# VideoVerses/VideoTuna-dev

Hardware: AMD Instinct MI355X
Metric: finetune samples/sec, CogVideoX-2B T2V LoRA 49x480x720 bf16 (higher is better)
Workload: dtype bf16; 1 GPU; CogVideoX-2B T2V LoRA finetune 49x480x720 (configs[1]): latents [4,13,16,60,90], text [4,226,4096], r=4 LoRA on to_q/k/v/out, 4 samples per optimizer step as in the YAML (batch_size 2 x accumulate_grad_batches 2), run as 1 micro-batch(es) of 4; mode=lora, model=CogVideoX-2B, micro_batch=4, accumulate_grad_batches=1, global_batch=4, seq_len=17776, layers=30, parallelism=dp1, recompute=none (107 GB of block activations kept in HBM), weights=seeded random init (no checkpoints offline), text=pre-encoded prompt embeddings (synthetic), latents=pre-encoded latents (synthetic)

## Files before the change

videotuna-dev_amd/csrc/gemm_bf16.hip:

```cpp
#include "gemm_epilogue.h"

#ifndef VT_SUFFIX
#define VT_SUFFIX
#endif
#ifndef VT_GEMM_DMA
#define VT_GEMM_DMA 1
#endif
#define VT_CAT_(a, b) a##b
#define VT_CAT(a, b) VT_CAT_(a, b)
#define GEMM_KERNEL VT_CAT(gemm_tn_kernel, VT_SUFFIX)
#define GEMM_ENTRY VT_CAT(vt_gemm_bf16, VT_SUFFIX)

#define BM 128
#define BN 128
#define BK 64
#define CS_LD 132

template <int EPI, bool OUT_F32>
__global__ __launch_bounds__(256, 2) void GEMM_KERNEL(GemmParams p) {
    __shared__ __attribute__((aligned(16))) char smem[65536];
    const int tid = threadIdx.x, lane = tid & 63, wave = tid >> 6;
    const int wm = wave & 1, wn = wave >> 1;
    const int nbm = (p.M + BM - 1) / BM, nbn = (p.N + BN - 1) / BN;
    const int id = xcd_remap(blockIdx.x, nbm * nbn);
    const int GM = 8;
    const int in_group = GM * nbn;
    const int group = id / in_group;
    const int first_m = group * GM;
    const int gsz = min(nbm - first_m, GM);
    const int tile_m = first_m + (id % in_group) % gsz;
    const int tile_n = (id % in_group) / gsz;
    const int row0 = tile_m * BM, col0 = tile_n * BN;

    const long long a_rem = (long long)(p.M - row0) * p.lda * 2;
    const long long w_rem = (long long)(p.N - col0) * p.ldw * 2;
    __amdgpu_buffer_rsrc_t ra = make_rsrc(p.A + (size_t)row0 * p.lda, (unsigned)(a_rem > 0x7fffffffLL ? 0x7fffffffLL : a_rem));
    __amdgpu_buffer_rsrc_t rw = make_rsrc(p.W + (size_t)col0 * p.ldw, (unsigned)(w_rem > 0x7fffffffLL ? 0x7fffffffLL : w_rem));

#if VT_GEMM_DMA
    const int wv = __builtin_amdgcn_readfirstlane(wave);
    const int drl = lane >> 3, dcp = lane & 7;
    int a_voff[4], w_voff[4];
#pragma unroll
    for (int j = 0; j < 4; ++j) {
        const int row = 8 * (wv + 4 * j) + drl;
        a_voff[j] = row * p.lda * 2 + ((dcp ^ drl) << 4);
        w_voff[j] = row * p.ldw * 2 + ((dcp ^ drl) << 4);
    }
    auto dma = [&](int kt, int buf) {
        const int soff = kt * BK * 2;
#pragma unroll
        for (int j = 0; j < 4; ++j) {
            char* dst = smem + buf * 32768 + (wv + 4 * j) * 1024;
            __builtin_amdgcn_raw_ptr_buffer_load_lds(ra, (__attribute__((address_space(3))) void*)dst, 16, a_voff[j], soff, 0, 0);
            __builtin_amdgcn_raw_ptr_buffer_load_lds(rw, (__attribute__((address_space(3))) void*)(dst + 16384), 16, w_voff[j], soff, 0, 0);
        }
    };
#else
    int a_voff[4], w_voff[4], lds_off[4];
#pragma unroll
    for (int j = 0; j < 4; ++j) {
        int i = tid + 256 * j;
        int r = i >> 3, c = i & 7;
        a_voff[j] = r * p.lda * 2 + c * 16;
        w_voff[j] = r * p.ldw * 2 + c * 16;
        lds_off[j] = r * 128 + ((c ^ (r & 7)) << 4);
    }
    u32x4 ga[4], gw[4];
    auto gload = [&](int kt) {
        const int soff = kt * BK * 2;
#pragma unroll
        for (int j = 0; j < 4; ++j) {
            ga[j] = __builtin_bit_cast(u32x4, __builtin_amdgcn_raw_buffer_load_b128(ra, a_voff[j], soff, 0));
            gw[j] = __builtin_bit_cast(u32x4, __builtin_amdgcn_raw_buffer_load_b128(rw, w_voff[j], soff, 0));
        }
    };
    auto lstore = [&](int buf) {
        char* base = smem + buf * 32768;
#pragma unroll
        for (int j = 0; j < 4; ++j) {
            *(u32x4*)(base + lds_off[j]) = ga[j];
            *(u32x4*)(base + 16384 + lds_off[j]) = gw[j];
        }
    };
#endif

    f32x4 acc[4][4];
#pragma unroll
    for (int i = 0; i < 4; ++i)
#pragma unroll
        for (int j = 0; j < 4; ++j) acc[i][j] = (f32x4){0.f, 0.f, 0.f, 0.f};

    const int nk = p.K / BK;
#if VT_GEMM_DMA
    dma(0, 0);
#else
    gload(0);
    lstore(0);
#endif
    __syncthreads();
    const int frow = lane & 15;
    const int fq = lane >> 4;
    const int fx = lane & 7;
    for (int kt = 0; kt < nk; ++kt) {
        const int buf = kt & 1;
#if VT_GEMM_DMA
        if (kt + 1 < nk) dma(kt + 1, buf ^ 1);
#else
        if (kt + 1 < nk) gload(kt + 1);
#endif
        const char* As = smem + buf * 32768;
        const char* Ws = As + 16384;
#pragma unroll
        for (int ks = 0; ks < 2; ++ks) {
            const int coff = (((ks * 4 + fq) ^ fx) << 4);
            bf16x8 af[4], wf[4];
#pragma unroll
            for (int t = 0; t < 4; ++t) {
                af[t] = *(const bf16x8*)(As + (wm * 64 + t * 16 + frow) * 128 + coff);
                wf[t] = *(const bf16x8*)(Ws + (wn * 64 + t * 16 + frow) * 128 + coff);
            }
#pragma unroll
            for (int tn = 0; tn < 4; ++tn)
#pragma unroll
                for (int tm = 0; tm < 4; ++tm)
                    acc[tn][tm] = __builtin_amdgcn_mfma_f32_16x16x32_bf16(wf[tn], af[tm], acc[tn][tm], 0, 0, 0);
        }
#if !VT_GEMM_DMA
        if (kt + 1 < nk) lstore(buf ^ 1);
#endif
        __syncthreads();
    }

    float* Cs = (float*)smem;
    const int er = tid >> 5;
    const int ec = (tid & 31) * 4;
    const int n = col0 + ec;
    float bias4[4] = {0.f, 0.f, 0.f, 0.f};
    if (p.bias != nullptr && n < p.N) {
#pragma unroll
        for (int j = 0; j < 4; ++j) bias4[j] = bf2f(p.bias[n + j]);
    }
#pragma unroll
    for (int half = 0; half < 2; ++half) {
        if (wm == half) {
#pragma unroll
            for (int tn = 0; tn < 4; ++tn)
#pragma unroll
                for (int tm = 0; tm < 4; ++tm) {
                    int ml = tm * 16 + frow;
                    int nl = wn * 64 + tn * 16 + fq * 4;
                    *(f32x4*)(Cs + ml * CS_LD + nl) = acc[tn][tm];
                }
        }
        __syncthreads();
#pragma unroll
        for (int pass = 0; pass < 8; ++pass) {
            const int ml = pass * 8 + er;
            const int m = row0 + half * 64 + ml;
            if (m < p.M && n < p.N) {
                f32x4 v = *(const f32x4*)(Cs + ml * CS_LD + ec);
                gemm_epilogue_store<EPI, OUT_F32>(p, m, n, v, bias4);
            }
        }
        __syncthreads();
    }
}

template <int EPI, bool F32>
static int VT_CAT(launch, VT_SUFFIX)(const GemmParams& p, hipStream_t st) {
    const int nbm = (p.M + BM - 1) / BM, nbn = (p.N + BN - 1) / BN;
    hipLaunchKernelGGL((GEMM_KERNEL<EPI, F32>), dim3(nbm * nbn), dim3(256), 0, st, p);
    return hipGetLastError() == hipSuccess ? VT_OK : VT_ERR_LAUNCH;
}

static bool VT_CAT(al16, VT_SUFFIX)(const void* p) { return (((uintptr_t)p) & 15) == 0; }

int VT_CAT(vt_gemm_big_dispatch, VT_SUFFIX)(const GemmParams& p, int epilogue, int out_fp32, hipStream_t st);
int VT_CAT(vt_gemm_pc_dispatch, VT_SUFFIX)(const GemmParams& p, int epilogue, int out_fp32, hipStream_t st);
static int VT_CAT(g_gemm_tile, VT_SUFFIX) = 0;
extern "C" int VT_CAT(vt_gemm_set_tile, VT_SUFFIX)(int mode) {
    if (mode < 0 || mode > 3) return VT_ERR_BAD_SHAPE;
    VT_CAT(g_gemm_tile, VT_SUFFIX) = mode;
    return VT_OK;
}
static int VT_CAT(pick_tile, VT_SUFFIX)(int M, int N, int K) {
    const int mode = VT_CAT(g_gemm_tile, VT_SUFFIX);
    if (mode) return mode;
    const long long t256 = (long long)((M + 255) / 256) * ((N + 255) / 256);
    const long long tpc = (long long)((M + 255) / 256) * ((N + 127) / 128);
    if (N >= 6144 && t256 >= 512) return 2;
    if (K >= 512 && M >= 1024) {
        const long long passes = (t256 + 255) / 256;
        const bool full = t256 <= 256 ? t256 >= 160 : 10 * t256 >= 9 * passes * 256;
        if (full && (N >= 2560 || ((N % 640) == 0 && N <= 1280) || ((N % 256) >= 192 && K >= 4096))) return 2;
    }
    if (tpc >= 512 && K >= 512) return 3;
    if (M > 64 && M <= 1024 && (long long)N * K >= (1LL << 24)) return 3;
    return 1;
}

int VT_CAT(vt_gemm_pc_bm, VT_SUFFIX)(int M);
extern "C" int VT_CAT(vt_gemm_bf16_kernel, VT_SUFFIX)(int M, int N, int K) {
    if (M <= 0 || N <= 0 || K <= 0) return VT_ERR_BAD_SHAPE;
    const int tile = VT_CAT(pick_tile, VT_SUFFIX)(M, N, K);
    return tile == 3 && VT_CAT(vt_gemm_pc_bm, VT_SUFFIX)(M) == 128 ? 4 : tile;
}

extern "C" int GEMM_ENTRY(const void* A, int lda, const void* W, int ldw, void* C, int ldc,
                            int M, int N, int K, const void* bias, int epilogue, int out_fp32,
                            const void* R, int ldr, int r_mod,
                            const float* gate_txt, const float* gate_vid, int gate_bstride, int S, int St,
                            void* C2, int ldc2, const void* U, int ldu, void* stream) {
    if (M <= 0 || N <= 0 || K <= 0 || (K % BK) != 0 || (N % 4) != 0) return VT_ERR_BAD_SHAPE;
    if ((lda % 8) || (ldw % 8) || (ldc % 4) || lda < K || ldw < K || ldc < N) return VT_ERR_BAD_SHAPE;
    if (!VT_CAT(al16, VT_SUFFIX)(A) || !VT_CAT(al16, VT_SUFFIX)(W) || !VT_CAT(al16, VT_SUFFIX)(C)) return VT_ERR_BAD_ALIGN;
    GemmParams p;
    p.A = (const bf16_t*)A; p.W = (const bf16_t*)W; p.C = C; p.bias = (const bf16_t*)bias;
    p.R = (const bf16_t*)R; p.gate_txt = gate_txt; p.gate_vid = gate_vid;
    p.C2 = (bf16_t*)C2; p.U = (const bf16_t*)U;
    p.M = M; p.N = N; p.K = K; p.lda = lda; p.ldw = ldw; p.ldc = ldc; p.ldr = ldr; p.ldc2 = ldc2; p.ldu = ldu;
    p.S = S > 0 ? S : 1; p.St = St; p.gate_bstride = gate_bstride; p.r_mod = r_mod; p.splits = 1;
    hipStream_t st = (hipStream_t)stream;
    const int tile = VT_CAT(pick_tile, VT_SUFFIX)(M, N, K);
    const bool big = tile == 2;
    if (tile == 3) {
        if (epilogue == EPI_BIAS_GELU && (out_fp32 || C2 == nullptr || (ldc2 % 4) || !VT_CAT(al16, VT_SUFFIX)(C2))) return VT_ERR_BAD_SHAPE;
        if (epilogue == EPI_GATED_RES && (out_fp32 || R == nullptr || (ldr % 4) || !VT_CAT(al16, VT_SUFFIX)(R))) return VT_ERR_BAD_SHAPE;
        if (epilogue == EPI_DGELU && (out_fp32 || U == nullptr || (ldu % 4) || !VT_CAT(al16, VT_SUFFIX)(U))) return VT_ERR_BAD_SHAPE;
        return VT_CAT(vt_gemm_pc_dispatch, VT_SUFFIX)(p, epilogue, out_fp32, st);
    }
    switch (epilogue) {
        case EPI_BIAS:
            if (big) return VT_CAT(vt_gemm_big_dispatch, VT_SUFFIX)(p, epilogue, out_fp32, st);
            return out_fp32 ? VT_CAT(launch, VT_SUFFIX)<EPI_BIAS, true>(p, st) : VT_CAT(launch, VT_SUFFIX)<EPI_BIAS, false>(p, st);
        case EPI_BIAS_GELU:
            if (out_fp32 || C2 == nullptr || (ldc2 % 4) || !VT_CAT(al16, VT_SUFFIX)(C2)) return VT_ERR_BAD_SHAPE;
            if (big) return VT_CAT(vt_gemm_big_dispatch, VT_SUFFIX)(p, epilogue, 0, st);
            return VT_CAT(launch, VT_SUFFIX)<EPI_BIAS_GELU, false>(p, st);
        case EPI_GATED_RES:
            if (out_fp32 || R == nullptr || (ldr % 4) || !VT_CAT(al16, VT_SUFFIX)(R)) return VT_ERR_BAD_SHAPE;
            if (C2 != nullptr && ((ldc2 % 4) || !VT_CAT(al16, VT_SUFFIX)(C2))) return VT_ERR_BAD_SHAPE;
            if (gate_vid != nullptr && (gate_txt == nullptr || (gate_bstride % 4) || !VT_CAT(al16, VT_SUFFIX)(gate_vid) || !VT_CAT(al16, VT_SUFFIX)(gate_txt)))
                return VT_ERR_BAD_SHAPE;
            if (big) return VT_CAT(vt_gemm_big_dispatch, VT_SUFFIX)(p, epilogue, 0, st);
            return VT_CAT(launch, VT_SUFFIX)<EPI_GATED_RES, false>(p, st);
        case EPI_DGELU:
            if (out_fp32 || U == nullptr || (ldu % 4) || !VT_CAT(al16, VT_SUFFIX)(U)) return VT_ERR_BAD_SHAPE;
            if (big) return VT_CAT(vt_gemm_big_dispatch, VT_SUFFIX)(p, epilogue, 0, st);
            return VT_CAT(launch, VT_SUFFIX)<EPI_DGELU, false>(p, st);
        default:
            return VT_ERR_UNSUPPORTED;
    }
}
```

videotuna-dev_amd/csrc/gemm_big_bf16.hip:

```cpp
#include "gemm_epilogue.h"

#ifndef VT_SUFFIX
#define VT_SUFFIX
#endif
#define VT_CAT_(a, b) a##b
#define VT_CAT(a, b) VT_CAT_(a, b)
#define GEMM_BIG_KERNEL VT_CAT(gemm_tn_big_kernel, VT_SUFFIX)
#define GEMM_BIG_ENTRY VT_CAT(vt_gemm_bf16_big, VT_SUFFIX)

#define GB_BM 256
#define GB_BN 256
#define GB_BK 64
#define GB_STAGE 65536
#ifndef GB_LOADERS
#define GB_LOADERS 0
#endif
#ifndef GB_STAGGER
#define GB_STAGGER 1
#endif
#ifndef GB_MFMA16
#define GB_MFMA16 1
#endif
#ifndef GB_W4
#define GB_W4 0
#endif
#define GB_THREADS (GB_LOADERS ? 768 : (GB_W4 ? 256 : 512))
#define GB_TN (GB_W4 ? 8 : 4)
#define GB_EROWS (GB_W4 ? 4 : 8)
#define GB_EPASS (32 / GB_EROWS)
#define GB_CS_LD 260

typedef int gb_i32x4 __attribute__((ext_vector_type(4)));

__device__ __forceinline__ void gb_lds_barrier() { asm volatile("s_waitcnt lgkmcnt(0)\n\ts_barrier" ::: "memory"); }

struct GbTile {
    int row0, col0;
    const bf16_t* a;
    const bf16_t* w;
    unsigned a_bytes, w_bytes;
};
__device__ __forceinline__ gb_i32x4 gb_words(const void* base, unsigned bytes) {
    const unsigned long long a = (unsigned long long)base;
    return (gb_i32x4){(int)(unsigned)a, (int)((a >> 32) & 0xffffu), (int)bytes, 0x00020000};
}

__device__ __forceinline__ GbTile gb_tile(const GemmParams& p, int id, int nbm, int nbn) {
    const int GM = 4;
    const int in_group = GM * nbn;
    const int group = id / in_group;
    const int first_m = group * GM;
    const int gsz = min(nbm - first_m, GM);
    GbTile t;
    t.row0 = (first_m + (id % in_group) % gsz) * GB_BM;
    t.col0 = ((id % in_group) / gsz) * GB_BN;
    const long long a_rem = (long long)(p.M - t.row0) * p.lda * 2;
    const long long w_rem = (long long)(p.N - t.col0) * p.ldw * 2;
    t.a = p.A + (size_t)t.row0 * p.lda;
    t.w = p.W + (size_t)t.col0 * p.ldw;
    t.a_bytes = (unsigned)(a_rem > 0x7fffffffLL ? 0x7fffffffLL : a_rem);
    t.w_bytes = (unsigned)(w_rem > 0x7fffffffLL ? 0x7fffffffLL : w_rem);
    return t;
}

template <int EPI, bool OUT_F32>
__global__ __launch_bounds__(GB_THREADS, 1) void GEMM_BIG_KERNEL(GemmParams p) {
    __shared__ __attribute__((aligned(16))) char smem[2 * GB_STAGE];
    const int tid = threadIdx.x, lane = tid & 63;
    const int wave = __builtin_amdgcn_readfirstlane(tid >> 6);
    const int wm = wave & 1, wn = wave >> 1;
    const int nbm = (p.M + GB_BM - 1) / GB_BM, nbn = (p.N + GB_BN - 1) / GB_BN;
    const int ntiles = nbm * nbn;
    const int spx = gridDim.x >> 3;
    const int slot = (int)(blockIdx.x & 7) * spx + (int)(blockIdx.x >> 3);
    const unsigned smem_lds = (unsigned)(uintptr_t)(__attribute__((address_space(3))) char*)smem;

    const int drl = lane >> 3, dcp = lane & 7;
#if GB_LOADERS
    const bool loader = wave >= 8;
    constexpr int NP = 8, PSTRIDE = 4;
    const int pw = wave & 3;
#else
    constexpr bool loader = true;
    constexpr int NP = GB_W4 ? 8 : 4, PSTRIDE = GB_W4 ? 4 : 8;
    const int pw = wave;
#endif
    const int row0p = 8 * pw + drl;
    const int sw = (row0p >> 1) & 7;
    const int a_voff0 = row0p * p.lda * 2 + ((dcp ^ sw) << 4);
    const int w_voff0 = row0p * p.ldw * 2 + ((dcp ^ sw) << 4);
    const int a_pstep = 8 * PSTRIDE * p.lda * 2, w_pstep = 8 * PSTRIDE * p.ldw * 2;
    auto dma = [&](const GbTile& t, int kt, int buf, int j0 = 0, int j1 = NP) {
        const int soff = kt * GB_BK * 2;
        __amdgpu_buffer_rsrc_t ra = make_rsrc(t.a, t.a_bytes), rw = make_rsrc(t.w, t.w_bytes);
#pragma unroll
        for (int j = j0; j < j1; ++j) {
            char* dst = smem + buf * GB_STAGE + (pw + PSTRIDE * j) * 1024;
            __builtin_amdgcn_raw_ptr_buffer_load_lds(ra, (__attribute__((address_space(3))) void*)dst, 16, a_voff0, soff + j * a_pstep, 0, 0);
            __builtin_amdgcn_raw_ptr_buffer_load_lds(rw, (__attribute__((address_space(3))) void*)(dst + 32768), 16, w_voff0, soff + j * w_pstep, 0, 0);
        }
    };
    auto dma_hidden = [&](const GbTile& t, int buf, int j0 = 0, int j1 = NP) {
        const gb_i32x4 ra = gb_words(t.a, t.a_bytes), rw = gb_words(t.w, t.w_bytes);
#pragma unroll
        for (int j = j0; j < j1; ++j) {
            const unsigned dst = smem_lds + buf * GB_STAGE + (pw + PSTRIDE * j) * 1024;
            asm volatile("s_mov_b32 m0, %0\n\ts_nop 0\n\tbuffer_load_dwordx4 %1, %2, %3 offen lds" :: "s"(dst), "v"(a_voff0), "s"(ra), "s"(j * a_pstep) : "memory");
            asm volatile("s_mov_b32 m0, %0\n\ts_nop 0\n\tbuffer_load_dwordx4 %1, %2, %3 offen lds" :: "s"(dst + 32768), "v"(w_voff0), "s"(rw), "s"(j * w_pstep) : "memory");
        }
    };

    const int nk = p.K / GB_BK;
    const int fr = lane & 31;
    const int fh = lane >> 5;
    const int fx = (fr >> 1) & 7;
    const int fr16 = lane & 15, fq = lane >> 4, fx16 = (fr16 >> 1) & 7;
    const int er = tid >> 6;
    const int ec = (tid & 63) * 4;

    if (slot >= ntiles) return;
    GbTile cur = gb_tile(p, slot, nbm, nbn);
    int buf = 0;
    if (loader) dma(cur, 0, 0);
    for (int tile = slot; tile < ntiles; tile += gridDim.x) {
        const bool has_next = tile + (int)gridDim.x < ntiles;
        GbTile nxt = cur;
        if (has_next) nxt = gb_tile(p, tile + gridDim.x, nbm, nbn);

#if GB_MFMA16
        f32x4 acc16[GB_TN][8];
#pragma unroll
        for (int i = 0; i < GB_TN; ++i)
#pragma unroll
            for (int j = 0; j < 8; ++j) acc16[i][j] = (f32x4){0.f, 0.f, 0.f, 0.f};
#else
        f32x16 acc[2][4];
#pragma unroll
        for (int i = 0; i < 2; ++i)
#pragma unroll
            for (int j = 0; j < 4; ++j)
#pragma unroll
                for (int e = 0; e < 16; ++e) acc[i][j][e] = 0.f;
#endif

        __syncthreads();
        for (int kt = 0; kt < nk; ++kt) {
            const bool last = kt + 1 == nk;
            auto issue = [&](int j0, int j1) {
#ifndef GB_ABL_NODMA
                if (loader) {
                    if (!last) dma(cur, kt + 1, buf ^ 1, j0, j1);
                    else if (has_next) dma_hidden(nxt, buf ^ 1, j0, j1);
                }
#endif
            };
            const bool late = GB_STAGGER && !GB_LOADERS && !GB_W4 && wave >= 4;
            if (GB_STAGGER < 2 && !late && !GB_W4) issue(0, NP);
#if GB_LOADERS
            if (!loader)
#endif
            {
#if GB_MFMA16
                const char* As = smem + buf * GB_STAGE + (wm * 128 + fr16) * 128;
                const char* Ws = smem + buf * GB_STAGE + 32768 + (wn * (16 * GB_TN) + fr16) * 128;
#pragma unroll
                for (int ks = 0; ks < 2; ++ks) {
                    if (GB_STAGGER == 1 && ks == 1 && late) issue(0, NP);
                    if (GB_STAGGER == 2 && !late) issue(2 * ks, 2 * ks + 2);
                    const int coff = (((ks * 4 + fq) ^ fx16) << 4);
                    bf16x8 af[8], wf[GB_TN];
#pragma unroll
                    for (int t = 0; t < 8; ++t) af[t] = *(const bf16x8*)(As + t * 2048 + coff);
#pragma unroll
                    for (int t = 0; t < GB_TN; ++t) wf[t] = *(const bf16x8*)(Ws + t * 2048 + coff);
#pragma unroll
                    for (int tm = 0; tm < 8; ++tm) {
                        if (GB_STAGGER == 2 && late && tm == 4) issue(2 * ks, 2 * ks + 2);
                        if (GB_W4 && !(tm & 1)) issue(4 * ks + (tm >> 1), 4 * ks + (tm >> 1) + 1);
#pragma unroll
                        for (int tn = 0; tn < GB_TN; ++tn)
                            acc16[tn][tm] = __builtin_amdgcn_mfma_f32_16x16x32_bf16(wf[tn], af[tm], acc16[tn][tm], 0, 0, 0);
                    }
                }
#else
                const char* As = smem + buf * GB_STAGE + (wm * 128 + fr) * 128;
                const char* Ws = smem + buf * GB_STAGE + 32768 + (wn * 64 + fr) * 128;
#pragma unroll
                for (int ks = 0; ks < 4; ++ks) {
                    if (GB_STAGGER == 1 && ks == 2 && late) issue(0, NP);
                    if (GB_STAGGER == 2 && !late) issue(ks, ks + 1);
                    const int coff = (((ks * 2 + fh) ^ fx) << 4);
                    bf16x8 af[4], wf[2];
#pragma unroll
                    for (int t = 0; t < 4; ++t) af[t] = *(const bf16x8*)(As + t * 4096 + coff);
#pragma unroll
                    for (int t = 0; t < 2; ++t) wf[t] = *(const bf16x8*)(Ws + t * 4096 + coff);
#pragma unroll
                    for (int tm = 0; tm < 4; ++tm) {
                        if (GB_STAGGER == 2 && late && tm == 2) issue(ks, ks + 1);
#pragma unroll
                        for (int tn = 0; tn < 2; ++tn)
                            acc[tn][tm] = __builtin_amdgcn_mfma_f32_32x32x16_bf16(wf[tn], af[tm], acc[tn][tm], 0, 0, 0);
                    }
                }
#endif
            }
#ifndef GB_ABL_NOBAR
            if (!last) __syncthreads();
            else gb_lds_barrier();
#endif
            buf ^= 1;
        }

        float* Cs = (float*)(smem + (buf ^ 1) * GB_STAGE);
        const int n = cur.col0 + ec;
        float bias4[4] = {0.f, 0.f, 0.f, 0.f};
        if (p.bias != nullptr && n < p.N) {
#pragma unroll
            for (int j = 0; j < 4; ++j) bias4[j] = bf2f(p.bias[n + j]);
        }
        constexpr bool HAS_AUX = EPI == EPI_GATED_RES || EPI == EPI_DGELU;
        u32x2 aux[GB_EPASS], auxn[GB_EPASS];
        auto aux_fetch = [&](int slab, u32x2* dst) {
#pragma unroll
            for (int pass = 0; pass < GB_EPASS; ++pass) {
                const int m = cur.row0 + slab * 32 + pass * GB_EROWS + er;
                dst[pass] = (u32x2){0u, 0u};
                if (HAS_AUX && wave < 8 && m < p.M && n < p.N) dst[pass] = gemm_epilogue_aux_load<EPI>(p, m, n);
            }
        };
        aux_fetch(0, aux);
        GateCtx gctx;
        if (EPI == EPI_GATED_RES) gctx = gate_ctx_load(p, cur.row0, GB_BM, n);
#pragma unroll
        for (int slab = 0; slab < 8; ++slab) {
            if (wave < 8 && wm == (slab >> 2)) {
#if GB_MFMA16
#pragma unroll
                for (int t2 = 0; t2 < 2; ++t2)
#pragma unroll
                    for (int tn = 0; tn < GB_TN; ++tn)
                        *(f32x4*)(Cs + (t2 * 16 + fr16) * GB_CS_LD + wn * (16 * GB_TN) + tn * 16 + 4 * fq) = acc16[tn][(slab & 3) * 2 + t2];
#else
                const int tm = slab & 3;
#pragma unroll
                for (int tn = 0; tn < 2; ++tn)
#pragma unroll
                    for (int q = 0; q < 4; ++q) {
                        const int nl = wn * 64 + tn * 32 + 8 * q + 4 * fh;
                        *(f32x4*)(Cs + fr * GB_CS_LD + nl) =
                            (f32x4){acc[tn][tm][4 * q], acc[tn][tm][4 * q + 1], acc[tn][tm][4 * q + 2], acc[tn][tm][4 * q + 3]};
                    }
#endif
            }
            gb_lds_barrier();
            if (slab < 7) aux_fetch(slab + 1, auxn);
#pragma unroll
            for (int pass = 0; pass < GB_EPASS; ++pass) {
                const int ml = pass * GB_EROWS + er;
                const int m = cur.row0 + slab * 32 + ml;
                if (wave < 8 && m < p.M && n < p.N) {
                    const f32x4 v = *(const f32x4*)(Cs + ml * GB_CS_LD + ec);
                    gemm_epilogue_store_aux<EPI, OUT_F32>(p, m, n, v, bias4, aux[pass], EPI == EPI_GATED_RES ? &gctx : nullptr);
                }
            }
            gb_lds_barrier();
#pragma unroll
            for (int pass = 0; pass < GB_EPASS; ++pass) aux[pass] = auxn[pass];
        }
        cur = nxt;
    }
}

template <int EPI, bool F32>
static int VT_CAT(launch_big, VT_SUFFIX)(const GemmParams& p, hipStream_t st) {
    const int nbm = (p.M + GB_BM - 1) / GB_BM, nbn = (p.N + GB_BN - 1) / GB_BN;
    static int slots = 0;
    if (slots == 0) {
        int dev = 0, cus = 0;
        if (hipGetDevice(&dev) != hipSuccess || hipDeviceGetAttribute(&cus, hipDeviceAttributeMultiprocessorCount, dev) != hipSuccess) cus = 0;
        slots = cus >= 8 ? cus / 8 * 8 : 8;
    }
    const int ntiles = nbm * nbn;
    const int grid = ntiles < slots ? (ntiles + 7) / 8 * 8 : slots;
    hipLaunchKernelGGL((GEMM_BIG_KERNEL<EPI, F32>), dim3(grid), dim3(GB_THREADS), 0, st, p);
    return hipGetLastError() == hipSuccess ? VT_OK : VT_ERR_LAUNCH;
}

int VT_CAT(vt_gemm_big_dispatch, VT_SUFFIX)(const GemmParams& p, int epilogue, int out_fp32, hipStream_t st) {
    switch (epilogue) {
        case EPI_BIAS:
            return out_fp32 ? VT_CAT(launch_big, VT_SUFFIX)<EPI_BIAS, true>(p, st) : VT_CAT(launch_big, VT_SUFFIX)<EPI_BIAS, false>(p, st);
        case EPI_BIAS_GELU: return VT_CAT(launch_big, VT_SUFFIX)<EPI_BIAS_GELU, false>(p, st);
        case EPI_GATED_RES: return VT_CAT(launch_big, VT_SUFFIX)<EPI_GATED_RES, false>(p, st);
        case EPI_DGELU: return VT_CAT(launch_big, VT_SUFFIX)<EPI_DGELU, false>(p, st);
        default: return VT_ERR_UNSUPPORTED;
    }
}
```

Baseline: 2.758 samples/s.

## Add phased quarter-tile DMA/MFMA pipeline to big GEMM and widen its selection

Replaces the big 256x256 GEMM main loop with a phased schedule. Each k-step is split into four MFMA quarters over A/W halves, and the buffer_load-to-LDS fetches for the next stages are interleaved between them under explicit barriers and vmcnt waits. Staggered waves are offset by one barrier. This aims to hide global-to-LDS latency and reduce full-block syncs. The dispatch heuristic also sends more N shapes with N%256>=128 and K<4096 to the big kernel. The hand-tuned wait counts and barrier pairing are fragile, and the fetch prefetches two stages ahead into a buffer being read.

Measured after the change: 2.782 samples/s (median of 6 runs). No clear change (+0.9%).

```diff
diff --git a/videotuna-dev_amd/csrc/gemm_bf16.hip b/videotuna-dev_amd/csrc/gemm_bf16.hip
--- a/videotuna-dev_amd/csrc/gemm_bf16.hip
+++ b/videotuna-dev_amd/csrc/gemm_bf16.hip
@@ -193,7 +193,8 @@
     if (K >= 512 && M >= 1024) {
         const long long passes = (t256 + 255) / 256;
         const bool full = t256 <= 256 ? t256 >= 160 : 10 * t256 >= 9 * passes * 256;
-        if (full && (N >= 2560 || ((N % 640) == 0 && N <= 1280) || ((N % 256) >= 192 && K >= 4096))) return 2;
+        if (full && (N >= 2560 || ((N % 640) == 0 && N <= 1280) || ((N % 256) >= 192 && K >= 4096) || ((N % 256) >= 128 && N >= 1920 && K < 4096)))
+            return 2;
     }
     if (tpc >= 512 && K >= 512) return 3;
     if (M > 64 && M <= 1024 && (long long)N * K >= (1LL << 24)) return 3;
diff --git a/videotuna-dev_amd/csrc/gemm_big_bf16.hip b/videotuna-dev_amd/csrc/gemm_big_bf16.hip
--- a/videotuna-dev_amd/csrc/gemm_big_bf16.hip
+++ b/videotuna-dev_amd/csrc/gemm_big_bf16.hip
@@ -24,6 +24,10 @@
 #ifndef GB_W4
 #define GB_W4 0
 #endif
+#ifndef GB_PHASED
+#define GB_PHASED 1
+#endif
+#define GB_PHASED_ON (GB_PHASED && GB_MFMA16 && !GB_W4 && !GB_LOADERS)
 #define GB_THREADS (GB_LOADERS ? 768 : (GB_W4 ? 256 : 512))
 #define GB_TN (GB_W4 ? 8 : 4)
 #define GB_EROWS (GB_W4 ? 4 : 8)
@@ -121,7 +125,37 @@
     if (slot >= ntiles) return;
     GbTile cur = gb_tile(p, slot, nbm, nbn);
     int buf = 0;
+#if GB_PHASED_ON
+    const int wpar = wave & 1, wq = wave >> 1;
+    const int wrow0 = 64 * wq + 8 * wpar + drl;
+    const int wsw = (wrow0 >> 1) & 7;
+    const int w_voffp = wrow0 * p.ldw * 2 + ((dcp ^ wsw) << 4);
+    const int w_step16 = 16 * p.ldw * 2;
+    const unsigned a_dst0 = smem_lds + wave * 1024, w_dst0 = smem_lds + 32768 + (8 * wq + wpar) * 1024;
+    auto stage_a = [&](const GbTile& t, int kt, int b, int hi) {
+        const gb_i32x4 ra = gb_words(t.a, t.a_bytes);
+#pragma unroll
+        for (int i = 0; i < 2; ++i) {
+            const int j = hi + 2 * i;
+            asm volatile("s_mov_b32 m0, %0\n\ts_nop 0\n\tbuffer_load_dwordx4 %1, %2, %3 offen lds"
+                         :: "s"(a_dst0 + b * GB_STAGE + j * 8192), "v"(a_voff0), "s"(ra), "s"(kt * (GB_BK * 2) + j * a_pstep) : "memory");
+        }
+    };
+    auto stage_w = [&](const GbTile& t, int kt, int b, int hi) {
+        const gb_i32x4 rw = gb_words(t.w, t.w_bytes);
+#pragma unroll
+        for (int i = 0; i < 2; ++i) {
+            const int j = 2 * hi + i;
+            asm volatile("s_mov_b32 m0, %0\n\ts_nop 0\n\tbuffer_load_dwordx4 %1, %2, %3 offen lds"
+                         :: "s"(w_dst0 + b * GB_STAGE + j * 2048), "v"(w_voffp), "s"(rw), "s"(kt * (GB_BK * 2) + j * w_step16) : "memory");
+        }
+    };
+    if (nk > 1) { stage_a(cur, 0, 0, 0); stage_w(cur, 0, 0, 0); }
+    stage_w(cur, 0, 0, 1);
+    stage_a(cur, 0, 0, 1);
+#else
     if (loader) dma(cur, 0, 0);
+#endif
     for (int tile = slot; tile < ntiles; tile += gridDim.x) {
         const bool has_next = tile + (int)gridDim.x < ntiles;
         GbTile nxt = cur;
@@ -143,6 +177,80 @@
                 for (int e = 0; e < 16; ++e) acc[i][j][e] = 0.f;
 #endif
 
+#if GB_PHASED_ON
+        const bool late = wave >= 4;
+        auto fetch_a = [&](int k, int b, int hi) {
+            if (k < nk) stage_a(cur, k, b, hi);
+            else if (k == nk && has_next) stage_a(nxt, 0, b, hi);
+        };
+        auto fetch_w = [&](int k, int b, int hi) {
+            if (k < nk) stage_w(cur, k, b, hi);
+            else if (k == nk && has_next) stage_w(nxt, 0, b, hi);
+        };
+        auto bar = [&]() { asm volatile("s_barrier" ::: "memory"); __builtin_amdgcn_sched_barrier(0); };
+        auto mma = [&](const bf16x8 (&a)[2][4], const bf16x8 (&w)[2][2], int tn0, int tm0) {
+            asm volatile("s_waitcnt lgkmcnt(0)" ::: "memory");
+            __builtin_amdgcn_sched_barrier(0);
+#pragma unroll
+            for (int ks = 0; ks < 2; ++ks)
+#pragma unroll
+                for (int tm = 0; tm < 4; ++tm)
+#pragma unroll
+                    for (int tn = 0; tn < 2; ++tn)
+                        acc16[tn0 + tn][tm0 + tm] = __builtin_amdgcn_mfma_f32_16x16x32_bf16(w[ks][tn], a[ks][tm], acc16[tn0 + tn][tm0 + tm], 0, 0, 0);
+            __builtin_amdgcn_sched_barrier(0);
+        };
+        if (nk == 1) { stage_a(cur, 0, buf, 0); stage_w(cur, 0, buf, 0); }
+        asm volatile("s_waitcnt vmcnt(0)" ::: "memory");
+        if (nk > 1) { stage_a(cur, 1, buf ^ 1, 0); stage_w(cur, 1, buf ^ 1, 0); }
+        bar();
+        if (late) bar();
+        const int coff0 = ((fq ^ fx16) << 4), coff1 = (((4 + fq) ^ fx16) << 4);
+        for (int kt = 0; kt < nk; ++kt) {
+            const bool drain = !has_next && kt + 2 >= nk;
+            auto wait = [&]() {
+                if (drain) asm volatile("s_waitcnt vmcnt(0)" ::: "memory");
+                else asm volatile("s_waitcnt vmcnt(8)" ::: "memory");
+                __builtin_amdgcn_sched_barrier(0);
+            };
+            const char* As = smem + buf * GB_STAGE + (wm * 128 + fr16) * 128;
+            const char* Ws = smem + buf * GB_STAGE + 32768 + (wn * 64 + fr16) * 128;
+            bf16x8 af[2][4], wlo[2][2], whi[2][2];
+#pragma unroll
+            for (int t = 0; t < 2; ++t) { wlo[0][t] = *(const bf16x8*)(Ws + t * 2048 + coff0); wlo[1][t] = *(const bf16x8*)(Ws + t * 2048 + coff1); }
+            __builtin_amdgcn_sched_barrier(0);
+#pragma unroll
+            for (int t = 0; t < 4; ++t) { af[0][t] = *(const bf16x8*)(As + t * 2048 + coff0); af[1][t] = *(const bf16x8*)(As + t * 2048 + coff1); }
+            __builtin_amdgcn_sched_barrier(0);
+            fetch_w(kt + 1, buf ^ 1, 1);
+            wait();
+            bar();
+            mma(af, wlo, 0, 0);
+            bar();
+#pragma unroll
+            for (int t = 0; t < 2; ++t) { whi[0][t] = *(const bf16x8*)(Ws + (2 + t) * 2048 + coff0); whi[1][t] = *(const bf16x8*)(Ws + (2 + t) * 2048 + coff1); }
+            __builtin_amdgcn_sched_barrier(0);
+            fetch_a(kt + 1, buf ^ 1, 1);
+            wait();
+            bar();
+            mma(af, whi, 2, 0);
+            bar();
+#pragma unroll
+            for (int t = 0; t < 4; ++t) { af[0][t] = *(const bf16x8*)(As + (4 + t) * 2048 + coff0); af[1][t] = *(const bf16x8*)(As + (4 + t) * 2048 + coff1); }
+            __builtin_amdgcn_sched_barrier(0);
+            fetch_a(kt + 2, buf, 0);
+            bar();
+            mma(af, whi, 2, 4);
+            bar();
+            fetch_w(kt + 2, buf, 0);
+            if (kt + 1 < nk) wait();
+            bar();
+            mma(af, wlo, 0, 4);
+            bar();
+            buf ^= 1;
+        }
+        if (!late) bar();
+#else
         __syncthreads();
         for (int kt = 0; kt < nk; ++kt) {
             const bool last = kt + 1 == nk;
@@ -211,6 +319,7 @@
 #endif
             buf ^= 1;
         }
+#endif
 
         float* Cs = (float*)(smem + (buf ^ 1) * GB_STAGE);
         const int n = cur.col0 + ec;
```
